# Sukikui/PTI-LDM-VAE

Measured on AMD Instinct MI355X. Metric: vae_train_images_per_sec_256x256, higher is better.
Workload: dtype fp16 forward operands + activations / bf16 backward operands + gradients, fp32 accumulate; 1 GPU; config/vae_dente_no_adv.json 256x256x1 batch 32/GPU: fwd + L1 + 1e-3*KL + bwd + all-reduce + Adam (perceptual term omitted: --perceptual times it; adversarial branch inactive before epoch 6, --adv times it); global_batch=32, parallelism=dp1

## Files before the change

### pti_ldm_vae_amd/csrc/wgrad_mfma.hip

```cpp
#include "pti_common.h"

namespace {

constexpr int TH = 8, TW = 16;
constexpr int PTI_WGRAD_SLAB_V4 = 1 << 30;
#ifndef PTI_WGRAD_BATCH_MAX
#define PTI_WGRAD_BATCH_MAX 16
#endif

struct WgArgs {
  const bf16* x;
  const bf16* dy;
  const stat_t* in_stats;
  const float* gamma;
  const float* beta;
  float* slab;
  int N, H, W, Cin, Ho, Wo, Cout;
  int mode, prologue, groups;
  float eps, inv_cnt;
  int tiles_x, tiles_y, ntiles, S;
  int ci_tiles;
  long long slab_stride;
  int x_f16;
  int diag;
};

template <int KS, int S_, int CO_T, int CI_T>
struct WCfg {
  static constexpr int HH = (TH - 1) * S_ + KS, HW = (TW - 1) * S_ + KS;
  static constexpr int NP = HH * HW;
  static constexpr int KK = KS * KS;
  static constexpr int PA = CI_T * 2 + (CI_T == 64 ? 64 : 0);
  static constexpr int PD = CO_T * 2 + (CO_T == 64 ? 64 : 0);
  static constexpr int NCA = CI_T / 8, NCD = CO_T / 8;
  static constexpr int WCO = CO_T / 32, WCI = CI_T / 32, WPX = 4 / (WCO * WCI);
  static constexpr int A_BYTES = NP * PA, D_BYTES = TH * TW * PD;
  static constexpr int HIT = (NP * NCA + 255) / 256, DIT = (TH * TW * NCD + 255) / 256;
  static constexpr int RED_BYTES = (WPX > 1) ? 32 * 32 * 4 * (WPX - 1) * WCO * WCI : 0;
  static constexpr int LDS_BYTES = (A_BYTES + D_BYTES) > RED_BYTES ? (A_BYTES + D_BYTES) : RED_BYTES;
};

template <int KS, int S_, int CO_T, int CI_T, bool PLAIN>
__global__ __launch_bounds__(256, 2) void wgrad_mfma_kernel(WgArgs a) {
  using C = WCfg<KS, S_, CO_T, CI_T>;
  const int prologue = PLAIN ? PTI_PRO_NONE : a.prologue;
  typedef short v4s __attribute__((ext_vector_type(4)));
  __shared__ __attribute__((aligned(16))) unsigned char smem[C::LDS_BYTES];
  unsigned char* lA = smem;
  unsigned char* lD = smem + C::A_BYTES;

  const int tid = threadIdx.x, lane = tid & 63, wave = tid >> 6;
  const int split = blockIdx.y;
  const int cot = blockIdx.x / a.ci_tiles, cit = blockIdx.x % a.ci_tiles;
  const int wco = wave / (C::WCI * C::WPX), wci = (wave / C::WPX) % C::WCI, wpx = wave % C::WPX;

  const int pad_lo = (a.mode == PTI_CONV_S2PAD) ? 0 : (KS - 1) / 2;
  const bool twox = (a.mode == PTI_CONV_UP2);
  const int VH = twox ? 2 * a.H : a.H, VW = twox ? 2 * a.W : a.W;

  const int g = lane >> 4, q = (lane & 15) >> 2, pp = lane & 3;
  const int pk = 8 * (g >> 1) + q;
  const int chl = 16 * (g & 1) + 4 * pp;
  const int dbase = pk * C::PD + (wco * 32 + chl) * 2;
  const int abase = (pk * S_) * C::PA + (wci * 32 + chl) * 2;

  f32x16 acc[C::KK];
#pragma unroll
  for (int t = 0; t < C::KK; ++t)
#pragma unroll
    for (int r = 0; r < 16; ++r) acc[t][r] = 0.f;

  const int alc = tid % C::NCA, alp = tid / C::NCA;
  constexpr int APSTEP = 256 / C::NCA;
  const int dlc = tid % C::NCD, dlp = tid / C::NCD;
  constexpr int DPSTEP = 256 / C::NCD;
  const int cpg = a.Cin / (a.groups > 0 ? a.groups : 1);
  float bsum[8];
#pragma unroll
  for (int j = 0; j < 8; ++j) bsum[j] = 0.f;

  u32x4 araw[C::HIT], draw[C::DIT];
  bool aok[C::HIT];
  int cur_n = -1;
  float sc[8], sh[8];

  auto issue_loads = [&](int tile) {
    int t = tile;
    const int tx_ = t % a.tiles_x; t /= a.tiles_x;
    const int ty_ = t % a.tiles_y;
    const int n = t / a.tiles_y;
    const int oy0 = ty_ * TH, ox0 = tx_ * TW;
    const int vy0 = oy0 * S_ - pad_lo, vx0 = ox0 * S_ - pad_lo;
#pragma unroll
    for (int it = 0; it < C::HIT; ++it) {
      const int p = alp + it * APSTEP;
      const int hy = p / C::HW, hx = p - hy * C::HW;
      const int vy = vy0 + hy, vx = vx0 + hx;
      const bool v = (p < C::NP) && vy >= 0 && vy < VH && vx >= 0 && vx < VW;
      const int iy = twox ? (vy >> 1) : vy, ix = twox ? (vx >> 1) : vx;
      aok[it] = v;
      araw[it] = u32x4{0u, 0u, 0u, 0u};
      if (v) araw[it] = *(const u32x4*)(a.x + ((size_t)(n * a.H + iy) * a.W + ix) * a.Cin + cit * CI_T + alc * 8);
    }
#pragma unroll
    for (int it = 0; it < C::DIT; ++it) {
      const int p = dlp + it * DPSTEP;
      const int ty = p / TW, tx = p % TW;
      const int oy = oy0 + ty, ox = ox0 + tx;
      draw[it] = u32x4{0u, 0u, 0u, 0u};
      if (p < TH * TW && oy < a.Ho && ox < a.Wo)
        draw[it] = *(const u32x4*)(a.dy + ((size_t)(n * a.Ho + oy) * a.Wo + ox) * a.Cout + cot * CO_T + dlc * 8);
    }
    return n;
  };

  auto write_lds = [&](int n) {
    if (prologue != PTI_PRO_NONE && n != cur_n) {
      cur_n = n;
#pragma unroll
      for (int j = 0; j < 8; ++j) {
        const int ch = cit * CI_T + alc * 8 + j;
        const int gg = ch / cpg;
        const float sum = stat_f(a.in_stats, (n * a.groups + gg) * 2), sq = stat_f(a.in_stats, (n * a.groups + gg) * 2 + 1);
        const float mean = sum * a.inv_cnt;
        const float rstd = rsqrtf(fmaxf(sq * a.inv_cnt - mean * mean, 0.f) + a.eps);
        sc[j] = rstd * a.gamma[ch];
        sh[j] = a.beta[ch] - mean * sc[j];
      }
    }
#pragma unroll
    for (int it = 0; it < C::HIT; ++it) {
      const int p = alp + it * APSTEP;
      if (p < C::NP) {
        u32x4 r = araw[it];
        if (prologue != PTI_PRO_NONE && aok[it]) {
          float f[8];
          unpack8f(r, f, a.x_f16);
#pragma unroll
          for (int j = 0; j < 8; ++j) {
            float v = f[j] * sc[j] + sh[j];
            if (prologue == PTI_PRO_GN_SILU) v = silu_f(v);
            f[j] = v;
          }
          r = pack8(f);
        } else if (a.x_f16) {
          float f[8];
          unpack8f(r, f, true);
          r = pack8(f);
        }
        *(u32x4*)(lA + p * C::PA + alc * 16) = r;
      }
    }
#pragma unroll
    for (int it = 0; it < C::DIT; ++it) {
      const int p = dlp + it * DPSTEP;
      if (p < TH * TW) {
        *(u32x4*)(lD + p * C::PD + dlc * 16) = draw[it];
        if (cit == 0) {
          float f[8];
          unpack8(draw[it], f);
#pragma unroll
          for (int j = 0; j < 8; ++j) bsum[j] += f[j];
        }
      }
    }
  };

  int tile = split;
  int n_next = -1;
  if (tile < a.ntiles) n_next = issue_loads(tile);
  for (; tile < a.ntiles; tile += a.S) {
    write_lds(n_next);
    __syncthreads();
    const int nxt = tile + a.S;
    if (nxt < a.ntiles) n_next = issue_loads(nxt);
#pragma unroll
    for (int rr = 0; rr < TH / C::WPX; ++rr) {
      const int row = wpx + rr * C::WPX;
      const unsigned char* dptr = lD + dbase + row * TW * C::PD;
      const v4s d0 = __builtin_amdgcn_ds_read_tr16_b64_v4i16((v4s __attribute__((address_space(3)))*)(dptr));
      const v4s d1 = __builtin_amdgcn_ds_read_tr16_b64_v4i16((v4s __attribute__((address_space(3)))*)(dptr + 4 * C::PD));
      bf16x8 dfrag;
      {
        typedef short v8s __attribute__((ext_vector_type(8)));
        v8s t8 = {d0[0], d0[1], d0[2], d0[3], d1[0], d1[1], d1[2], d1[3]};
        dfrag = __builtin_bit_cast(bf16x8, t8);
      }
#pragma unroll
      for (int kh = 0; kh < KS; ++kh) {
#pragma unroll
        for (int kw = 0; kw < KS; ++kw) {
          const unsigned char* aptr = lA + abase + ((row * S_ + kh) * C::HW + kw) * C::PA;
          const v4s a0 = __builtin_amdgcn_ds_read_tr16_b64_v4i16((v4s __attribute__((address_space(3)))*)(aptr));
          const v4s a1 = __builtin_amdgcn_ds_read_tr16_b64_v4i16((v4s __attribute__((address_space(3)))*)(aptr + 4 * S_ * C::PA));
          typedef short v8s __attribute__((ext_vector_type(8)));
          v8s t8 = {a0[0], a0[1], a0[2], a0[3], a1[0], a1[1], a1[2], a1[3]};
          const bf16x8 afrag = __builtin_bit_cast(bf16x8, t8);
          acc[kh * KS + kw] = __builtin_amdgcn_mfma_f32_32x32x16_bf16(dfrag, afrag, acc[kh * KS + kw], 0, 0, 0);
        }
      }
    }
    __syncthreads();
  }

  float* slab = a.slab + (size_t)split * a.slab_stride;
  const int ci = cit * CI_T + wci * 32 + (lane & 31);
  const int hsel = lane >> 5;
  float* red = reinterpret_cast<float*>(smem);
#pragma unroll
  for (int t = 0; t < C::KK; ++t) {
    if constexpr (C::WPX > 1) {
      if (wpx > 0) {
        float* dst = red + (((wco * C::WCI + wci) * (C::WPX - 1) + (wpx - 1)) * 16) * 64;
#pragma unroll
        for (int r = 0; r < 16; ++r) dst[r * 64 + lane] = acc[t][r];
      }
      __syncthreads();
      if (wpx == 0) {
#pragma unroll
        for (int o = 0; o < C::WPX - 1; ++o) {
          const float* src = red + (((wco * C::WCI + wci) * (C::WPX - 1) + o) * 16) * 64;
#pragma unroll
          for (int r = 0; r < 16; ++r) acc[t][r] += src[r * 64 + lane];
        }
      }
      __syncthreads();
    }
    if (wpx == 0) {
#pragma unroll
      for (int r = 0; r < 16; ++r) {
        const int co = cot * CO_T + wco * 32 + (r & 3) + 8 * (r >> 2) + 4 * hsel;
        slab[((size_t)t * a.Cout + co) * a.Cin + ci] = acc[t][r];
      }
    }
  }
  if (cit == 0) {
    __syncthreads();
#pragma unroll
    for (int j = 0; j < 8; ++j) red[j * 256 + tid] = bsum[j];
    __syncthreads();
    if (tid < CO_T) {
      const int lc = tid / 8, j = tid % 8;
      float s = 0.f;
      for (int k = lc; k < 256; k += C::NCD) s += red[j * 256 + k];
      slab[(size_t)C::KK * a.Cout * a.Cin + cot * CO_T + tid] = s;
    }
  }
}

template <int COB>
struct W3Cfg {
  static constexpr int TH = 8, HH = TH + 2, HW = TW + 2, NP = HH * HW;
  static constexpr int PP = 64;
  static constexpr int A_BYTES = NP * PP, DP_BYTES = TH * TW * PP;
  static constexpr int D_BYTES = COB * DP_BYTES;
  static constexpr int NT = 192;
  static constexpr int DPC = 4 * COB;
  static constexpr int HIT = (NP * 4 + NT - 1) / NT, DIT = (TH * TW * DPC + NT - 1) / NT;
  static constexpr int LDS_BYTES = A_BYTES + D_BYTES;
};

template <int COB, bool PLAIN>
__global__ __launch_bounds__(192) __attribute__((amdgpu_waves_per_eu(COB == 1 ? (PLAIN ? 4 : 3) : 2, COB == 1 ? (PLAIN ? 4 : 3) : 2)))
void wgrad_mfma3_kernel(WgArgs a) {
  using C = W3Cfg<COB>;
  const int prologue = PLAIN ? PTI_PRO_NONE : a.prologue;
  const bool x_f16 = (bool)a.x_f16;
  typedef short v4s __attribute__((ext_vector_type(4)));
  typedef short v8s __attribute__((ext_vector_type(8)));
  __shared__ __attribute__((aligned(16))) unsigned char smem[C::LDS_BYTES];
  unsigned char* lA = smem;
  unsigned char* lD = smem + C::A_BYTES;
  const int tid = threadIdx.x, lane = tid & 63, kw = tid >> 6;
  int split, cc;
  {
    const int id = blockIdx.x, tiles_cc = a.ci_tiles * (a.Cout / (32 * COB));
    if (a.S >= 8) {
      const int k = id >> 3;
      cc = k % tiles_cc;
      split = (k / tiles_cc) * 8 + (id & 7);
    } else {
      cc = id / a.S;
      split = id % a.S;
    }
  }
  const int cot = cc / a.ci_tiles, cit = cc % a.ci_tiles;
  const int co0 = cot * 32 * COB;
  const bool twox = (a.mode == PTI_CONV_UP2);
  const int VH = twox ? 2 * a.H : a.H, VW = twox ? 2 * a.W : a.W;

  const int g = lane >> 4, q = (lane & 15) >> 2, pp = lane & 3;
  const int pk = 8 * (g >> 1) + q, chl = 16 * (g & 1) + 4 * pp;
  const int fbase = pk * C::PP + chl * 2;

  f32x16 acc[COB][3];
#pragma unroll
  for (int h = 0; h < COB; ++h)
#pragma unroll
    for (int t = 0; t < 3; ++t)
#pragma unroll
      for (int r = 0; r < 16; ++r) acc[h][t][r] = 0.f;
  float bsum[8];
#pragma unroll
  for (int j = 0; j < 8; ++j) bsum[j] = 0.f;

  const int lc = tid & 3, lp = tid >> 2;
  const int lcd = tid % C::DPC, lpd = tid / C::DPC;
  constexpr int PSTEP = C::NT / 4, DSTEP = C::NT / C::DPC;
  const int cpg = a.Cin / (a.groups > 0 ? a.groups : 1);
  int cur_n = -1;
  float sc[8], sh[8];
  u32x4 araw[C::HIT], draw[C::DIT];
  unsigned aokm = 0;

  auto issue = [&](int tile) -> int {
    int t = tile;
    const int tx_ = t % a.tiles_x; t /= a.tiles_x;
    const int ty_ = t % a.tiles_y;
    const int n = t / a.tiles_y;
    const int oy0 = ty_ * C::TH, ox0 = tx_ * TW;
#pragma unroll
    for (int it = 0; it < C::HIT; ++it) {
      const int p = lp + it * PSTEP;
      const int hy = p / C::HW, hx = p - hy * C::HW;
      const int vy = oy0 - 1 + hy, vx = ox0 - 1 + hx;
      const bool v = (p < C::NP) && vy >= 0 && vy < VH && vx >= 0 && vx < VW;
      const int iy = twox ? (vy >> 1) : vy, ix = twox ? (vx >> 1) : vx;
      aokm = (aokm & ~(1u << it)) | ((unsigned)v << it);
      araw[it] = u32x4{0u, 0u, 0u, 0u};
      if (v) araw[it] = *(const u32x4*)(a.x + ((size_t)(n * a.H + iy) * a.W + ix) * a.Cin + cit * 32 + lc * 8);
    }
#pragma unroll
    for (int it = 0; it < C::DIT; ++it) {
      const int p = lpd + it * DSTEP;
      const int oy = oy0 + p / TW, ox = ox0 + p % TW;
      draw[it] = u32x4{0u, 0u, 0u, 0u};
      if (p < C::TH * TW && oy < a.Ho && ox < a.Wo)
        draw[it] = *(const u32x4*)(a.dy + ((size_t)(n * a.Ho + oy) * a.Wo + ox) * a.Cout + co0 + lcd * 8);
    }
    return n;
  };
  auto commit = [&](int n) {
    if (prologue != PTI_PRO_NONE && n != cur_n) {
      cur_n = n;
#pragma unroll
      for (int j = 0; j < 8; ++j) {
        const int ch = cit * 32 + lc * 8 + j;
        const int gg = ch / cpg;
        const float sum = stat_f(a.in_stats, (n * a.groups + gg) * 2), sq = stat_f(a.in_stats, (n * a.groups + gg) * 2 + 1);
        const float mean = sum * a.inv_cnt;
        const float rstd = rsqrtf(fmaxf(sq * a.inv_cnt - mean * mean, 0.f) + a.eps);
        sc[j] = rstd * a.gamma[ch];
        sh[j] = a.beta[ch] - mean * sc[j];
      }
    }
#pragma unroll
    for (int it = 0; it < C::HIT; ++it) {
      const int p = lp + it * PSTEP;
      if (p < C::NP) {
        u32x4 r = araw[it];
        if (prologue != PTI_PRO_NONE && ((aokm >> it) & 1u)) {
          float f[8];
          unpack8f(r, f, x_f16);
#pragma unroll
          for (int j = 0; j < 8; ++j) {
            float v = f[j] * sc[j] + sh[j];
            if (prologue == PTI_PRO_GN_SILU) v = silu_f(v);
            f[j] = v;
          }
          r = pack8(f);
        } else if (x_f16) {
          float f[8];
          unpack8f(r, f, true);
          r = pack8(f);
        }
        *(u32x4*)(lA + p * C::PP + lc * 16) = r;
      }
    }
#pragma unroll
    for (int it = 0; it < C::DIT; ++it) {
      const int p = lpd + it * DSTEP;
      if (p < C::TH * TW) {
        *(u32x4*)(lD + (lcd >> 2) * C::DP_BYTES + p * C::PP + (lcd & 3) * 16) = draw[it];
        if (cit == 0) {
          float f[8];
          unpack8(draw[it], f);
#pragma unroll
          for (int j = 0; j < 8; ++j) bsum[j] += f[j];
        }
      }
    }
  };

  int tile = split, n_next = -1;
  if (tile < a.ntiles) n_next = issue(tile);
  for (; tile < a.ntiles; tile += a.S) {
    commit(n_next);
    __syncthreads();
    const int nxt = tile + a.S;
    if (nxt < a.ntiles) n_next = issue(nxt);
// ... 771 lines not shown
#pragma unroll
    for (int r = 0; r < 4; ++r) dfr[r] = dnx[r];
    ps = ns;
  }
  wait_vmcnt<0>();

  const int ci = lane & 31, hsel = lane >> 5;
  if (do_bias) bsum += __shfl_xor(bsum, 32, 64);
  if constexpr (C::NRG == 2) {
    __syncthreads();
    float* red = reinterpret_cast<float*>(smem) + (cb + C::NCB * ch) * 5120;
    float* bred = reinterpret_cast<float*>(smem) + C::NCB * C::NCH * 5120;
#pragma unroll
    for (int round = 0; round < 2; ++round) {
      if (round) __syncthreads();
      if (rg == 1) {
#pragma unroll
        for (int t = 0; t < 9; ++t)
          if ((t < 5) == (round == 0))
#pragma unroll
            for (int q4 = 0; q4 < 4; ++q4)
              *(f32x4*)(red + (t - 5 * round) * 1024 + ci * 32 + (((2 * q4 + hsel) ^ (ci & 7)) << 2)) =
                  f32x4{acc[t / 3][t % 3][4 * q4], acc[t / 3][t % 3][4 * q4 + 1], acc[t / 3][t % 3][4 * q4 + 2], acc[t / 3][t % 3][4 * q4 + 3]};
        if (round == 0 && do_bias && lane < 32) bred[cb * 32 + lane] = bsum;
      }
      __syncthreads();
      if (rg == 0) {
#pragma unroll
        for (int t = 0; t < 9; ++t)
          if ((t < 5) == (round == 0))
#pragma unroll
            for (int q4 = 0; q4 < 4; ++q4) {
              const f32x4 v = *(const f32x4*)(red + (t - 5 * round) * 1024 + ci * 32 + (((2 * q4 + hsel) ^ (ci & 7)) << 2));
#pragma unroll
              for (int j = 0; j < 4; ++j) acc[t / 3][t % 3][4 * q4 + j] += v[j];
            }
        if (round == 0 && do_bias && lane < 32) bsum += bred[cb * 32 + lane];
      }
    }
    if (rg == 1) return;
  }
  const int cc32 = (C::NCB * cotb + cb) * (a.Cin / 32) + C::NCH * citb + ch;
  float* blk = a.slab + (size_t)split * a.slab_stride + (size_t)cc32 * 9216;
#pragma unroll
  for (int kh = 0; kh < 3; ++kh)
#pragma unroll
    for (int kw = 0; kw < 3; ++kw)
#pragma unroll
      for (int q4 = 0; q4 < 4; ++q4)
        *(f32x4*)(blk + (kh * 3 + kw) * 1024 + ci * 32 + (((2 * q4 + hsel) ^ (ci & 7)) << 2)) =
            f32x4{acc[kh][kw][4 * q4], acc[kh][kw][4 * q4 + 1], acc[kh][kw][4 * q4 + 2], acc[kh][kw][4 * q4 + 3]};
  if (do_bias && lane < 32) a.slab[(size_t)split * a.slab_stride + (size_t)9 * a.Cout * a.Cin + co0 + cb * 32 + lane] = bsum;
}

__global__ __launch_bounds__(256) void wgrad_reduce4_kernel(W4Batch b) {
  __shared__ f32x4 red[16][16];
  int jb = 0;
  while (jb + 1 < b.njobs && (int)blockIdx.x >= b.first_rblk[jb + 1]) ++jb;
  const W4Job& a = b.job[jb];
  const float* __restrict__ slab = a.slab;
  float* __restrict__ dw = b.dw[jb];
  float* __restrict__ dbias = b.dbias[jb];
  const int S = a.S, Cout = a.Cout, Cin = a.Cin, accumulate = b.accumulate[jb];
  const long long stride = a.slab_stride;
  const long long total = (long long)9 * Cout * Cin;
  const int col = threadIdx.x & 15, sg = threadIdx.x >> 4;
  const long long e = ((long long)(blockIdx.x - b.first_rblk[jb]) * 16 + col) * 4;
  f32x4 s0 = {0.f, 0.f, 0.f, 0.f}, s1 = s0;
  if (e < total + Cout) {
    int k = sg;
    for (; k + 16 < S; k += 32) {
      s0 += *(const f32x4*)(slab + (size_t)k * stride + e);
      s1 += *(const f32x4*)(slab + (size_t)(k + 16) * stride + e);
    }
    if (k < S) s0 += *(const f32x4*)(slab + (size_t)k * stride + e);
  }
  red[sg][col] = s0 + s1;
  __syncthreads();
  if (sg == 0 && e < total + Cout) {
    f32x4 sum = red[0][col];
#pragma unroll
    for (int g = 1; g < 16; ++g) sum += red[g][col];
    if (e < total) {
      const int cc = (int)(e / 9216), i = (int)(e % 9216);
      const int ci_tiles = Cin / 32;
      const int co0 = (cc / ci_tiles) * 32, ci0 = (cc % ci_tiles) * 32;
      const int tap = i >> 10, ci = (i >> 5) & 31, cog = ((i >> 2) & 7) ^ (ci & 7);
#pragma unroll
      for (int j = 0; j < 4; ++j) {
        const size_t o = ((size_t)(co0 + cog * 4 + j) * Cin + ci0 + ci) * 9 + tap;
        dw[o] = accumulate ? dw[o] + sum[j] : sum[j];
      }
    } else if (dbias) {
      const int co = (int)(e - total);
#pragma unroll
      for (int j = 0; j < 4; ++j) dbias[co + j] = accumulate ? dbias[co + j] + sum[j] : sum[j];
    }
  }
}

__global__ __launch_bounds__(256) void wgrad_reduce_kernel(const float* __restrict__ slab, long long stride, int S,
                                                           float* __restrict__ dw, float* __restrict__ dbias, int Cout,
                                                           int Cin, int KK, int accumulate) {
  __shared__ f32x4 red[16][16];
  const long long total = (long long)KK * Cout * Cin;
  const int col = threadIdx.x & 15, sg = threadIdx.x >> 4;
  const long long e = ((long long)blockIdx.x * 16 + col) * 4;
  f32x4 s0 = {0.f, 0.f, 0.f, 0.f}, s1 = s0;
  if (e < total + Cout) {
    int k = sg;
    for (; k + 16 < S; k += 32) {
      s0 += *(const f32x4*)(slab + (size_t)k * stride + e);
      s1 += *(const f32x4*)(slab + (size_t)(k + 16) * stride + e);
    }
    if (k < S) s0 += *(const f32x4*)(slab + (size_t)k * stride + e);
  }
  red[sg][col] = s0 + s1;
  __syncthreads();
  if (sg == 0 && e < total + Cout) {
    f32x4 sum = red[0][col];
#pragma unroll
    for (int g = 1; g < 16; ++g) sum += red[g][col];
    if (e < total) {
      const int ci = e % Cin;
      const int co = (e / Cin) % Cout;
      const int t = e / ((long long)Cin * Cout);
#pragma unroll
      for (int j = 0; j < 4; ++j) {
        const size_t o = ((size_t)co * Cin + ci + j) * KK + t;
        dw[o] = accumulate ? dw[o] + sum[j] : sum[j];
      }
    } else if (dbias) {
      const int co = (int)(e - total);
#pragma unroll
      for (int j = 0; j < 4; ++j) dbias[co + j] = accumulate ? dbias[co + j] + sum[j] : sum[j];
    }
  }
}

template <int KS, int S_, int CO_T, int CI_T>
void launch_w(const WgArgs& a, int grid_y, hipStream_t st) {
  if (a.prologue == PTI_PRO_NONE)
    PTI_LAUNCH((wgrad_mfma_kernel<KS, S_, CO_T, CI_T, true>), dim3(grid_y, a.S), dim3(256), 0, st, a);
  else
    PTI_LAUNCH((wgrad_mfma_kernel<KS, S_, CO_T, CI_T, false>), dim3(grid_y, a.S), dim3(256), 0, st, a);
}
template <int KS, int S_>
void launch_wt(const WgArgs& a, int co_t, int ci_t, int grid_y, hipStream_t st) {
  if (co_t == 64 && ci_t == 64) launch_w<KS, S_, 64, 64>(a, grid_y, st);
  else if (co_t == 64) launch_w<KS, S_, 64, 32>(a, grid_y, st);
  else if (ci_t == 64) launch_w<KS, S_, 32, 64>(a, grid_y, st);
  else launch_w<KS, S_, 32, 32>(a, grid_y, st);
}

}

static int w6_mode(int n, int h, int w, int cin, int cout) {
  const char* e = getenv("PTI_WGRAD_V6");
  const int v = e ? atoi(e) : 3;
  if (v >= 1 && cout % 128 == 0 && cin % 64 == 0) return 2;
  if (v >= 2 && cout % 64 == 0 && cin % 64 == 0 && (v == 2 || (long long)h * w <= 128 * 128)) return 3;
  return 0;
}
static void w4_fill_job(W4Job& a, const void* x, const void* dy, int n, int h, int w, int cin, int cout, int mode) {
  a.x = (const bf16*)x; a.dy = (const bf16*)dy; a.slab = nullptr;
  a.N = n; a.H = h; a.W = w; a.Cin = cin; a.Cout = cout;
  a.tiles_x = cdiv(w, TW); a.tiles_y = cdiv(h, mode == 2 ? W6A::TH_ : TH); a.ntiles = n * a.tiles_x * a.tiles_y;
  a.slab_stride = (long long)9 * cout * cin + cout;
  a.S = 1;
  a.cob2 = mode;
}
static bool w4_eligible(int n, int h, int w, int cin, int cout) {
  return n > 0 && h > 0 && w > 0 && cin > 0 && cout > 0 && cin % 32 == 0 && cout % 32 == 0 &&
         (long long)n * h * w * cin * 2 < (1ll << 31) && (long long)n * h * w * cout * 2 < (1ll << 31);
}
static int w4_mode(int cout) {
  static const int cob2_env = getenv("PTI_WGRAD_V4_COB2") ? atoi(getenv("PTI_WGRAD_V4_COB2")) : 1;
  return (cob2_env && cout % 64 == 0) ? 1 : 0;
}
extern "C" int pti_conv_wgrad_batched_mode(int n, int h, int w, int cin, int cout) {
  if (!w4_eligible(n, h, w, cin, cout)) return PTI_EUNSUPPORTED;
  const int v4 = w4_mode(cout), v6 = w6_mode(n, h, w, cin, cout);
  return v6 ? v6 : v4;
}
static int wgrad_diag_env() {
  const char* v = getenv("PTI_WGRAD_V4_DIAG");
  const char* ok = getenv("PTI_ALLOW_WRONG_RESULTS");
  if (!v || atoi(v) == 0) return 0;
  if (!ok || atoi(ok) != 1) {
    fprintf(stderr, "[pti] PTI_WGRAD_V4_DIAG ignored: it needs PTI_ALLOW_WRONG_RESULTS=1 (results are garbage)\n");
    return 0;
  }
  fprintf(stderr, "[pti] WRONG-RESULT DIAGNOSTIC ACTIVE: PTI_WGRAD_V4_DIAG=%s\n", v);
  return atoi(v);
}
static long long w4_plan(W4Batch& b, float* workspace, long long workspace_floats) {
  static const int wgs_env = getenv("PTI_WGRAD_V4_WGS") ? atoi(getenv("PTI_WGRAD_V4_WGS")) : 2048;
  static const int diag_env = wgrad_diag_env();
  b.diag = diag_env;
  auto tiles32 = [](const W4Job& a) {
    return a.cob2 == 2 ? (a.Cin / 64) * (a.Cout / 128) : a.cob2 == 3 ? (a.Cin / 64) * (a.Cout / 64)
                                                                     : (a.Cin / 32) * (a.Cout / (a.cob2 ? 64 : 32));
  };
  const bool m6 = b.njobs > 0 && b.job[0].cob2 >= 2;
  const char* w6e = getenv("PTI_WGRAD_V6_WGS");
  const int wgs6 = w6e && atoi(w6e) > 0 ? atoi(w6e) : 512;
  double work = 0;
  for (int j = 0; j < b.njobs; ++j) work += (double)tiles32(b.job[j]) * (b.job[j].cob2 == 1 ? 2 : 1) * b.job[j].ntiles;
  double per_wg = work / wgs_env > 2.0 ? work / wgs_env : 2.0;
  if (m6) per_wg = work / wgs6 > 4.0 ? work / wgs6 : 4.0;
  for (int attempt = 0;; ++attempt) {
    long long used = 0;
    int rb = 0, groups = 0;
    bool fits = true;
    for (int j = 0; j < b.njobs; ++j) {
      W4Job& a = b.job[j];
      int S = (int)((double)a.ntiles * (a.cob2 == 1 ? 2 : 1) / per_wg + 0.5);
      if (S > a.ntiles / (a.cob2 ? 1 : 2)) S = a.ntiles / (a.cob2 ? 1 : 2);
      if (S > 255) S = 255;
      if (S < 1) S = 1;
      if (used + (long long)S * a.slab_stride > workspace_floats) fits = false;
      a.S = S;
      a.slab = workspace + used;
      used += (long long)S * a.slab_stride;
      groups += S;
      b.first_rblk[j] = rb;
      rb += (int)((a.slab_stride / 4 + 15) / 16);
    }
    b.first_rblk[b.njobs] = rb;
    if (fits && groups <= 8 * W4_MAXGRP) {
      int len[8] = {0, 0, 0, 0, 0, 0, 0, 0};
      for (int x = 0; x < 8; ++x) { b.ngrp[x] = 0; b.grp_start[x][0] = 0; }
      int order[PTI_WGRAD_BATCH_MAX];
      for (int j = 0; j < b.njobs; ++j) order[j] = j;
      for (int i = 0; i < b.njobs; ++i)
        for (int j = i + 1; j < b.njobs; ++j)
          if (tiles32(b.job[order[j]]) > tiles32(b.job[order[i]])) { const int t = order[i]; order[i] = order[j]; order[j] = t; }
      bool ok = true;
      for (int i = 0; i < b.njobs && ok; ++i) {
        const int j = order[i];
        for (int sp = 0; sp < b.job[j].S; ++sp) {
          int best = 0;
          for (int x = 1; x < 8; ++x)
            if (len[x] < len[best]) best = x;
          if (b.ngrp[best] >= W4_MAXGRP || len[best] + tiles32(b.job[j]) > 65535) { ok = false; break; }
          b.grp[best][b.ngrp[best]] = (unsigned short)((unsigned)j | ((unsigned)sp << 4));
          len[best] += tiles32(b.job[j]);
          b.grp_start[best][++b.ngrp[best]] = (unsigned short)len[best];
        }
      }
      if (ok) {
        int mx = 0;
        for (int x = 0; x < 8; ++x) mx = len[x] > mx ? len[x] : mx;
        b.nwg = 8 * mx;
        return used;
      }
    }
    if (attempt > 40) return -1;
    per_wg *= 1.25;
  }
}

extern "C" int64_t pti_conv_wgrad_workspace_bytes(int cout, int cin, int ksize, int splits) {
  return (int64_t)splits * ((int64_t)ksize * ksize * cout * cin + cout) * 4;
}

static int wgrad_check(const void* x, const void* dy, const int64_t* in_stats, const float* gamma, const float* beta,
                       const void* workspace, const pti_conv_desc* d) {
  if (!x || !dy || !workspace || !d) PTI_FAIL(PTI_EINVAL, "conv_wgrad_mfma: null pointer");
  if (d->cin % 32 || d->cout % 32) PTI_FAIL(PTI_EUNSUPPORTED, "conv_wgrad_mfma: cin=%d cout=%d", d->cin, d->cout);
  if (d->ksize != 1 && d->ksize != 3) PTI_FAIL(PTI_EUNSUPPORTED, "conv_wgrad_mfma: ksize");
  if (d->mode == PTI_CONV_ZINS || (d->ksize == 1 && d->mode != PTI_CONV_S1)) PTI_FAIL(PTI_EUNSUPPORTED, "conv_wgrad_mfma: mode %d", d->mode);
  if (d->prologue != PTI_PRO_NONE && (!in_stats || !gamma || !beta || d->groups <= 0 || d->cin % d->groups))
    PTI_FAIL(PTI_EINVAL, "conv_wgrad_mfma: prologue args");
  return PTI_OK;
}

extern "C" int pti_conv_wgrad_mfma_partials(const void* x, const void* dy, const int64_t* in_stats, const float* gamma,
                                            const float* beta, void* workspace, int64_t workspace_bytes,
                                            const pti_conv_desc* d, int* splits_out, pti_stream_t s) {
  if (!splits_out) PTI_FAIL(PTI_EINVAL, "conv_wgrad_mfma_partials: null splits_out");
  if (int rc = wgrad_check(x, dy, in_stats, gamma, beta, workspace, d)) return rc;
  WgArgs a;
  a.x = (const bf16*)x; a.dy = (const bf16*)dy; a.in_stats = (const stat_t*)in_stats; a.gamma = gamma; a.beta = beta;
  a.slab = (float*)workspace;
  a.N = d->n; a.H = d->h; a.W = d->w; a.Cin = d->cin; a.Ho = d->ho; a.Wo = d->wo; a.Cout = d->cout;
  a.mode = d->mode; a.prologue = d->prologue; a.groups = d->groups; a.eps = d->eps; a.x_f16 = d->in_f16;
  static const int diag_env = wgrad_diag_env();
  a.diag = diag_env;
  a.inv_cnt = d->prologue != PTI_PRO_NONE ? 1.0f / ((float)(d->cin / d->groups) * (float)d->h * (float)d->w) : 0.f;
  a.tiles_x = cdiv(d->wo, TW); a.tiles_y = cdiv(d->ho, TH); a.ntiles = d->n * a.tiles_x * a.tiles_y;
  int co_t = d->cout % 64 == 0 ? 64 : 32, ci_t = d->cin % 64 == 0 ? 64 : 32;
  if ((long long)a.ntiles * (d->cout / co_t) * (d->cin / ci_t) < 16 * 512) co_t = ci_t = 32;
  const bool v3 = d->ksize == 3 && d->mode != PTI_CONV_S2PAD;
  static const int cob_env = getenv("PTI_WGRAD_COB") ? atoi(getenv("PTI_WGRAD_COB")) : 0;
  const bool cob_ok = d->cout % 64 == 0 && d->mode == PTI_CONV_S1;
  const int cob = (cob_ok && cob_env != 1 && (cob_env == 2 || d->prologue != PTI_PRO_NONE)) ? 2 : 1;
  if (v3) { ci_t = 32; co_t = 32 * cob; }
  a.ci_tiles = d->cin / ci_t;
  const int tiles_cc = (d->cout / co_t) * a.ci_tiles;
  const int kk = d->ksize * d->ksize;
  a.slab_stride = (long long)kk * d->cout * d->cin + d->cout;
  const long long smax = workspace_bytes / (a.slab_stride * 4);
  const bool plain = d->prologue == PTI_PRO_NONE && cob == 1;
  static const int v1_wgs = getenv("PTI_WGRAD_V1_WGS") ? atoi(getenv("PTI_WGRAD_V1_WGS")) : 512;
  int S = (v3 ? (cob == 2 ? 512 : (plain ? (tiles_cc == 1 ? 1024 : 1280) : 768)) : v1_wgs) / tiles_cc;
  if (S > a.ntiles / 4) S = a.ntiles / 4;
  const int scap = v3 ? (plain ? 1024 : 512) : 256;
  if (S > scap) S = scap;
  if (S < 1) S = 1;
  if (S > smax) S = (int)smax;
  if (S < 1) PTI_FAIL(PTI_EINVAL, "conv_wgrad_mfma: workspace too small (%lld bytes per split needed)", a.slab_stride * 4);
  static const int v4_env = getenv("PTI_WGRAD_V4") ? atoi(getenv("PTI_WGRAD_V4")) : 1;
  const bool v4 = v3 && v4_env && d->prologue == PTI_PRO_NONE && !d->in_f16 && d->mode == PTI_CONV_S1 &&
                  w4_eligible(d->n, d->h, d->w, d->cin, d->cout);
  if (v4) {
    W4Batch b;
    b.njobs = 1;
    w4_fill_job(b.job[0], x, dy, d->n, d->h, d->w, d->cin, d->cout, pti_conv_wgrad_batched_mode(d->n, d->h, d->w, d->cin, d->cout));
    b.dw[0] = b.dbias[0] = nullptr;
    b.accumulate[0] = 0;
    if (w4_plan(b, (float*)workspace, workspace_bytes / 4) < 0)
      PTI_FAIL(PTI_EINVAL, "conv_wgrad_mfma: workspace too small (%lld bytes per split needed)", a.slab_stride * 4);
    const char* v5e = getenv("PTI_WGRAD_V5");
    const bool v5 = v5e && atoi(v5e) != 0 && !b.diag;
    if (b.job[0].cob2 == 2) PTI_LAUNCH(wgrad_mfma6_kernel<W6A>, dim3(b.nwg), dim3(512), 0, (hipStream_t)s, b);
    else if (b.job[0].cob2 == 3) PTI_LAUNCH(wgrad_mfma6_kernel<W6B>, dim3(b.nwg), dim3(512), 0, (hipStream_t)s, b);
    else if (b.job[0].cob2 && v5) PTI_LAUNCH(wgrad_mfma5_kernel, dim3(b.nwg), dim3(256), 0, (hipStream_t)s, b);
    else if (b.job[0].cob2) PTI_LAUNCH(wgrad_mfma4_kernel<true>, dim3(b.nwg), dim3(512), 0, (hipStream_t)s, b);
    else PTI_LAUNCH(wgrad_mfma4_kernel<false>, dim3(b.nwg), dim3(512), 0, (hipStream_t)s, b);
    PTI_CHECK_LAUNCH("conv_wgrad_mfma");
    *splits_out = b.job[0].S | PTI_WGRAD_SLAB_V4;
    return PTI_OK;
  }
  if (v3 && S >= 8) S &= ~7;
  a.S = S;
  hipStream_t st = (hipStream_t)s;
  if (v3 && cob == 2) PTI_LAUNCH((wgrad_mfma3_kernel<2, false>), dim3(tiles_cc * S), dim3(192), 0, st, a);
  else if (v3 && plain) PTI_LAUNCH((wgrad_mfma3_kernel<1, true>), dim3(tiles_cc * S), dim3(192), 0, st, a);
  else if (v3) PTI_LAUNCH((wgrad_mfma3_kernel<1, false>), dim3(tiles_cc * S), dim3(192), 0, st, a);
  else if (d->ksize == 1) launch_wt<1, 1>(a, co_t, ci_t, tiles_cc, st);
  else launch_wt<3, 2>(a, co_t, ci_t, tiles_cc, st);
  PTI_CHECK_LAUNCH("conv_wgrad_mfma");
  *splits_out = S;
  return PTI_OK;
}

extern "C" int pti_conv_wgrad_reduce(const void* workspace, int splits, float* dw, float* dbias, int accumulate,
                                     const pti_conv_desc* d, pti_stream_t s) {
  if (!workspace || !dw || !d || splits < 1) PTI_FAIL(PTI_EINVAL, "conv_wgrad_reduce: bad arguments");
  const int kk = d->ksize * d->ksize;
  const long long total = (long long)kk * d->cout * d->cin + d->cout;
  if (splits & PTI_WGRAD_SLAB_V4) {
    if (kk != 9 || !w4_eligible(d->n, d->h, d->w, d->cin, d->cout)) PTI_FAIL(PTI_EINVAL, "conv_wgrad_reduce: block-ordered slabs are 3x3 only");
    W4Batch b;
    b.njobs = 1;
    w4_fill_job(b.job[0], nullptr, nullptr, d->n, d->h, d->w, d->cin, d->cout, w4_mode(d->cout));
    b.job[0].S = splits & ~PTI_WGRAD_SLAB_V4;
    b.job[0].slab = (float*)workspace;
    b.dw[0] = dw; b.dbias[0] = dbias; b.accumulate[0] = accumulate;
    b.diag = 0; b.nwg = 0;
    for (int x = 0; x < 8; ++x) b.ngrp[x] = 0;
    b.first_rblk[0] = 0;
    b.first_rblk[1] = (int)((total / 4 + 15) / 16);
    PTI_LAUNCH(wgrad_reduce4_kernel, dim3(b.first_rblk[1]), dim3(256), 0, (hipStream_t)s, b);
    PTI_CHECK_LAUNCH("conv_wgrad_reduce");
    return PTI_OK;
  }
  PTI_LAUNCH(wgrad_reduce_kernel, dim3((unsigned)((total / 4 + 15) / 16)), dim3(256), 0, (hipStream_t)s,
                     (const float*)workspace, total, splits, dw, dbias, d->cout, d->cin, kk, accumulate);
  PTI_CHECK_LAUNCH("conv_wgrad_reduce");
  return PTI_OK;
}

extern "C" int pti_conv_wgrad_mfma(const void* x, const void* dy, const int64_t* in_stats, const float* gamma,
                                   const float* beta, float* dw, float* dbias, void* workspace,
                                   int64_t workspace_bytes, int accumulate, const pti_conv_desc* d, pti_stream_t s) {
  if (!dw) PTI_FAIL(PTI_EINVAL, "conv_wgrad_mfma: null pointer");
  int splits = 0;
  if (int rc = pti_conv_wgrad_mfma_partials(x, dy, in_stats, gamma, beta, workspace, workspace_bytes, d, &splits, s)) return rc;
  return pti_conv_wgrad_reduce(workspace, splits, dw, dbias, accumulate, d, s);
}

extern "C" int pti_conv_wgrad_mfma_batched(const pti_wgrad_job* jobs, int njobs, void* workspace, int64_t workspace_bytes,
                                           pti_stream_t s) {
  if (!jobs || !workspace || njobs < 1 || njobs > PTI_WGRAD_BATCH_MAX)
    PTI_FAIL(PTI_EINVAL, "conv_wgrad_mfma_batched: 1..%d jobs", PTI_WGRAD_BATCH_MAX);
  W4Batch bm[4];
  bm[0].njobs = bm[1].njobs = bm[2].njobs = bm[3].njobs = 0;
  for (int j = 0; j < njobs; ++j) {
    const pti_wgrad_job& q = jobs[j];
    if (!q.x || !q.dy || !q.dw) PTI_FAIL(PTI_EINVAL, "conv_wgrad_mfma_batched: job %d has a null pointer", j);
    const int mode = pti_conv_wgrad_batched_mode(q.n, q.h, q.w, q.cin, q.cout);
    if (mode < 0)
      PTI_FAIL(PTI_EUNSUPPORTED, "conv_wgrad_mfma_batched: job %d: n=%d h=%d w=%d cin=%d cout=%d (channels must be multiples of 32, tensors < 2 GiB)",
               j, q.n, q.h, q.w, q.cin, q.cout);
    W4Job jb;
    w4_fill_job(jb, q.x, q.dy, q.n, q.h, q.w, q.cin, q.cout, mode);
    W4Batch& b = bm[mode];
    const int k = b.njobs++;
    b.job[k] = jb;
    b.dw[k] = q.dw; b.dbias[k] = q.dbias; b.accumulate[k] = q.accumulate;
  }
  float* ws = (float*)workspace;
  long long ws_floats = workspace_bytes / 4;
  const char* v5e = getenv("PTI_WGRAD_V5");
  const int v5_env = v5e ? atoi(v5e) : 0;
  const void* main_kernel = nullptr;
  long long need[4] = {0, 0, 0, 0}, need_all = 0;
  for (int m = 0; m < 4; ++m) {
    for (int j = 0; j < bm[m].njobs; ++j) need[m] += bm[m].job[j].slab_stride;
    need_all += need[m];
  }
  if (need_all > ws_floats) PTI_FAIL(PTI_EINVAL, "conv_wgrad_mfma_batched: workspace too small (%lld bytes needed for one split per job)", need_all * 4);
  const long long ws_total = ws_floats;
  for (int m = 3; m >= 0; --m) {
    W4Batch& b = bm[m];
    if (b.njobs == 0) continue;
    long long later = 0;
    for (int m2 = m - 1; m2 >= 0; --m2) later += need[m2];
    long long avail = (long long)((double)ws_total * ((double)need[m] / (double)need_all));
    if (avail < need[m]) avail = need[m];
    if (later == 0 || avail > ws_floats - later) avail = ws_floats - later;
    const long long used = w4_plan(b, ws, avail);
    if (used < 0) PTI_FAIL(PTI_EINVAL, "conv_wgrad_mfma_batched: workspace too small");
    ws += used;
    ws_floats -= used;
    const void* kfn;
    if (m == 3) { PTI_LAUNCH(wgrad_mfma6_kernel<W6B>, dim3(b.nwg), dim3(512), 0, (hipStream_t)s, b); kfn = reinterpret_cast<const void*>(wgrad_mfma6_kernel<W6B>); }
    else if (m == 2) { PTI_LAUNCH(wgrad_mfma6_kernel<W6A>, dim3(b.nwg), dim3(512), 0, (hipStream_t)s, b); kfn = reinterpret_cast<const void*>(wgrad_mfma6_kernel<W6A>); }
    else if (m == 1 && v5_env && !b.diag) { PTI_LAUNCH(wgrad_mfma5_kernel, dim3(b.nwg), dim3(256), 0, (hipStream_t)s, b); kfn = reinterpret_cast<const void*>(wgrad_mfma5_kernel); }
    else if (m == 1) { PTI_LAUNCH(wgrad_mfma4_kernel<true>, dim3(b.nwg), dim3(512), 0, (hipStream_t)s, b); kfn = reinterpret_cast<const void*>(wgrad_mfma4_kernel<true>); }
    else { PTI_LAUNCH(wgrad_mfma4_kernel<false>, dim3(b.nwg), dim3(512), 0, (hipStream_t)s, b); kfn = reinterpret_cast<const void*>(wgrad_mfma4_kernel<false>); }
    PTI_CHECK_LAUNCH("conv_wgrad_mfma_batched");
    if (!main_kernel) main_kernel = kfn;
    PTI_LAUNCH(wgrad_reduce4_kernel, dim3(b.first_rblk[b.njobs]), dim3(256), 0, (hipStream_t)s, b);
    PTI_CHECK_LAUNCH("conv_wgrad_mfma_batched reduce");
  }
  pti_last_kernel = main_kernel;
  return PTI_OK;
}
```

Baseline: 2739 images/s.

## Add dedicated 1x1 weight-gradient kernel with pixel-linear tiles and larger channel tiles

```diff
diff --git a/pti_ldm_vae_amd/csrc/wgrad_mfma.hip b/pti_ldm_vae_amd/csrc/wgrad_mfma.hip
--- a/pti_ldm_vae_amd/csrc/wgrad_mfma.hip
+++ b/pti_ldm_vae_amd/csrc/wgrad_mfma.hip
@@ -1,3 +1,5 @@
+#include <algorithm>
+
 #include "pti_common.h"
 
 namespace {
@@ -41,7 +43,7 @@
 };
 
 template <int KS, int S_, int CO_T, int CI_T, bool PLAIN>
-__global__ __launch_bounds__(256, 2) void wgrad_mfma_kernel(WgArgs a) {
+__device__ __forceinline__ void wgrad_v1_body(const WgArgs& a) {
   using C = WCfg<KS, S_, CO_T, CI_T>;
   const int prologue = PLAIN ? PTI_PRO_NONE : a.prologue;
   typedef short v4s __attribute__((ext_vector_type(4)));
@@ -246,6 +248,229 @@
       slab[(size_t)C::KK * a.Cout * a.Cin + cot * CO_T + tid] = s;
     }
   }
+}
+
+constexpr int w1_tile_pixels(int co_t, int ci_t) { return co_t + ci_t <= 128 ? 128 : (co_t + ci_t <= 320 ? 64 : 32); }
+
+template <int CO_T, int CI_T>
+struct W1Cfg {
+  static constexpr int NBCO = CO_T / 32, NBCI = CI_T / 32;
+  static constexpr int WCO = (NBCO >= 4 && NBCI == 1) ? 4 : (NBCO >= 2 ? 2 : 1);
+  static constexpr int WCI = (NBCI >= 4 && NBCO == 1) ? 4 : (NBCI >= 2 ? 2 : 1);
+  static constexpr int WPX = 4 / (WCO * WCI);
+  static constexpr int BCO = NBCO / WCO, BCI = NBCI / WCI;
+  static constexpr int P = w1_tile_pixels(CO_T, CI_T);
+  static constexpr int NCA = CI_T / 8, NCD = CO_T / 8;
+  static constexpr int AIT = P * NCA / 256, DIT = P * NCD / 256;
+  static constexpr int skew(int nb) { return nb >= 4 ? 64 : (nb == 2 ? 128 : 0); }
+  static constexpr int SUBX = P * 64 + skew(NBCI), SUBD = P * 64 + skew(NBCO);
+  static constexpr int X_BYTES = NBCI * SUBX, D_BYTES = NBCO * SUBD;
+  static constexpr int RED_BYTES = (WPX > 1) ? 32 * 32 * 4 * (WPX - 1) * WCO * WCI : 0;
+  static constexpr int BIAS_BYTES = 8 * 256 * 4;
+  static constexpr int TILE_BYTES = X_BYTES + D_BYTES;
+  static constexpr int LDS_BYTES = TILE_BYTES > (RED_BYTES > BIAS_BYTES ? RED_BYTES : BIAS_BYTES)
+                                       ? TILE_BYTES : (RED_BYTES > BIAS_BYTES ? RED_BYTES : BIAS_BYTES);
+  static_assert(WCO * WCI * WPX == 4 && BCO * WCO == NBCO && BCI * WCI == NBCI, "wave layout");
+  static_assert(WPX == 1 || (BCO == 1 && BCI == 1), "waves split pixels only when each holds one block");
+  static_assert(P % (16 * WPX) == 0 && (P * NCA) % 256 == 0 && (P * NCD) % 256 == 0 && 256 % NCA == 0 && 256 % NCD == 0,
+                "loader geometry");
+};
+
+template <int CO_T, int CI_T, bool PLAIN>
+__device__ __forceinline__ void wgrad_1x1_body(const WgArgs& a) {
+  using C = W1Cfg<CO_T, CI_T>;
+  const int prologue = PLAIN ? PTI_PRO_NONE : a.prologue;
+  typedef short v4s __attribute__((ext_vector_type(4)));
+  typedef short v8s __attribute__((ext_vector_type(8)));
+  __shared__ __attribute__((aligned(16))) unsigned char smem[C::LDS_BYTES];
+  unsigned char* lX = smem;
+  unsigned char* lD = smem + C::X_BYTES;
+
+  const int tid = threadIdx.x, lane = tid & 63, wave = tid >> 6;
+  const int split = blockIdx.y;
+  const int cot = blockIdx.x / a.ci_tiles, cit = blockIdx.x % a.ci_tiles;
+  const int wco = wave / (C::WCI * C::WPX), wci = (wave / C::WPX) % C::WCI, wpx = wave % C::WPX;
+  const int HW = a.H * a.W;
+  const int tps = a.tiles_x;
+  const int t0 = (int)((long long)split * a.ntiles / a.S), t1 = (int)((long long)(split + 1) * a.ntiles / a.S);
+
+  const int g = lane >> 4, q = (lane & 15) >> 2, pp = lane & 3;
+  const int fbase = (8 * (g >> 1) + q) * 64 + (16 * (g & 1) + 4 * pp) * 2;
+
+  f32x16 acc[C::BCO * C::BCI];
+#pragma unroll
+  for (int b = 0; b < C::BCO * C::BCI; ++b)
+#pragma unroll
+    for (int r = 0; r < 16; ++r) acc[b][r] = 0.f;
+
+  constexpr int APSTEP = 256 / C::NCA, DPSTEP = 256 / C::NCD;
+  const int alc = tid % C::NCA, alp = tid / C::NCA;
+  const int dlc = tid % C::NCD, dlp = tid / C::NCD;
+  const bf16* xg = a.x + cit * CI_T + alc * 8;
+  const bf16* dg = a.dy + cot * CO_T + dlc * 8;
+  unsigned char* xl = lX + (alc >> 2) * C::SUBX + (alc & 3) * 16 + alp * 64;
+  unsigned char* dl = lD + (dlc >> 2) * C::SUBD + (dlc & 3) * 16 + dlp * 64;
+  const int cpg = a.Cin / (a.groups > 0 ? a.groups : 1);
+  float bsum[8];
+#pragma unroll
+  for (int j = 0; j < 8; ++j) bsum[j] = 0.f;
+
+  u32x4 araw[C::AIT], draw[C::DIT];
+  int cur_n = -1, n_next = -1, valid_next = 0;
+  float sc[8], sh[8];
+
+  auto issue_loads = [&](int tile) {
+    const int n = tile / tps, p0 = (tile - n * tps) * C::P;
+    const int valid = min(C::P, HW - p0);
+    const size_t pix0 = (size_t)n * HW + p0;
+#pragma unroll
+    for (int it = 0; it < C::AIT; ++it) {
+      const int p = alp + it * APSTEP;
+      araw[it] = u32x4{0u, 0u, 0u, 0u};
+      if (p < valid) araw[it] = *(const u32x4*)(xg + (pix0 + p) * a.Cin);
+    }
+#pragma unroll
+    for (int it = 0; it < C::DIT; ++it) {
+      const int p = dlp + it * DPSTEP;
+      draw[it] = u32x4{0u, 0u, 0u, 0u};
+      if (p < valid) draw[it] = *(const u32x4*)(dg + (pix0 + p) * a.Cout);
+    }
+    n_next = n;
+    valid_next = valid;
+  };
+
+  auto write_lds = [&]() {
+    if (prologue != PTI_PRO_NONE && n_next != cur_n) {
+      cur_n = n_next;
+#pragma unroll
+      for (int j = 0; j < 8; ++j) {
+        const int ch = cit * CI_T + alc * 8 + j;
+        const int gg = ch / cpg;
+        const float sum = stat_f(a.in_stats, (cur_n * a.groups + gg) * 2), sq = stat_f(a.in_stats, (cur_n * a.groups + gg) * 2 + 1);
+        const float mean = sum * a.inv_cnt;
+        const float rstd = rsqrtf(fmaxf(sq * a.inv_cnt - mean * mean, 0.f) + a.eps);
+        sc[j] = rstd * a.gamma[ch];
+        sh[j] = a.beta[ch] - mean * sc[j];
+      }
+    }
+#pragma unroll
+    for (int it = 0; it < C::AIT; ++it) {
+      u32x4 r = araw[it];
+      if (prologue != PTI_PRO_NONE) {
+        if (alp + it * APSTEP < valid_next) {
+          float f[8];
+          unpack8f(r, f, a.x_f16);
+#pragma unroll
+          for (int j = 0; j < 8; ++j) {
+            float v = f[j] * sc[j] + sh[j];
+            if (prologue == PTI_PRO_GN_SILU) v = silu_f(v);
+            f[j] = v;
+          }
+          r = pack8(f);
+        }
+      } else if (a.x_f16) {
+        float f[8];
+        unpack8f(r, f, true);
+        r = pack8(f);
+      }
+      *(u32x4*)(xl + it * APSTEP * 64) = r;
+    }
+#pragma unroll
+    for (int it = 0; it < C::DIT; ++it) {
+      *(u32x4*)(dl + it * DPSTEP * 64) = draw[it];
+      if (cit == 0) {
+        float f[8];
+        unpack8(draw[it], f);
+#pragma unroll
+        for (int j = 0; j < 8; ++j) bsum[j] += f[j];
+      }
+    }
+  };
+
+  if (t0 < t1) issue_loads(t0);
+  for (int tile = t0; tile < t1; ++tile) {
+    write_lds();
+    __syncthreads();
+    if (tile + 1 < t1) issue_loads(tile + 1);
+#pragma unroll
+    for (int ks = 0; ks < C::P / 16 / C::WPX; ++ks) {
+      const int poff = (ks * C::WPX + wpx) * 16 * 64 + fbase;
+      bf16x8 dfrag[C::BCO], xfrag[C::BCI];
+#pragma unroll
+      for (int i = 0; i < C::BCO; ++i) {
+        const unsigned char* ptr = lD + (wco * C::BCO + i) * C::SUBD + poff;
+        const v4s d0 = __builtin_amdgcn_ds_read_tr16_b64_v4i16((v4s __attribute__((address_space(3)))*)(ptr));
+        const v4s d1 = __builtin_amdgcn_ds_read_tr16_b64_v4i16((v4s __attribute__((address_space(3)))*)(ptr + 4 * 64));
+        const v8s t8 = {d0[0], d0[1], d0[2], d0[3], d1[0], d1[1], d1[2], d1[3]};
+        dfrag[i] = __builtin_bit_cast(bf16x8, t8);
+      }
+#pragma unroll
+      for (int j = 0; j < C::BCI; ++j) {
+        const unsigned char* ptr = lX + (wci * C::BCI + j) * C::SUBX + poff;
+        const v4s x0 = __builtin_amdgcn_ds_read_tr16_b64_v4i16((v4s __attribute__((address_space(3)))*)(ptr));
+        const v4s x1 = __builtin_amdgcn_ds_read_tr16_b64_v4i16((v4s __attribute__((address_space(3)))*)(ptr + 4 * 64));
+        const v8s t8 = {x0[0], x0[1], x0[2], x0[3], x1[0], x1[1], x1[2], x1[3]};
+        xfrag[j] = __builtin_bit_cast(bf16x8, t8);
+      }
+#pragma unroll
+      for (int i = 0; i < C::BCO; ++i)
+#pragma unroll
+        for (int j = 0; j < C::BCI; ++j)
+          acc[i * C::BCI + j] = __builtin_amdgcn_mfma_f32_32x32x16_bf16(dfrag[i], xfrag[j], acc[i * C::BCI + j], 0, 0, 0);
+    }
+    __syncthreads();
+  }
+
+  float* slab = a.slab + (size_t)split * a.slab_stride;
+  const int hsel = lane >> 5;
+  float* red = reinterpret_cast<float*>(smem);
+  if constexpr (C::WPX > 1) {
+    if (wpx > 0) {
+      float* dst = red + (((wco * C::WCI + wci) * (C::WPX - 1) + (wpx - 1)) * 16) * 64;
+#pragma unroll
+      for (int r = 0; r < 16; ++r) dst[r * 64 + lane] = acc[0][r];
+    }
+    __syncthreads();
+    if (wpx == 0) {
+#pragma unroll
+      for (int o = 0; o < C::WPX - 1; ++o) {
+        const float* src = red + (((wco * C::WCI + wci) * (C::WPX - 1) + o) * 16) * 64;
+#pragma unroll
+        for (int r = 0; r < 16; ++r) acc[0][r] += src[r * 64 + lane];
+      }
+    }
+  }
+  if (wpx == 0) {
+#pragma unroll
+    for (int i = 0; i < C::BCO; ++i)
+#pragma unroll
+      for (int j = 0; j < C::BCI; ++j) {
+        const int ci = cit * CI_T + (wci * C::BCI + j) * 32 + (lane & 31);
+#pragma unroll
+        for (int r = 0; r < 16; ++r) {
+          const int co = cot * CO_T + (wco * C::BCO + i) * 32 + (r & 3) + 8 * (r >> 2) + 4 * hsel;
+          slab[(size_t)co * a.Cin + ci] = acc[i * C::BCI + j][r];
+        }
+      }
+  }
+  if (cit == 0) {
+    __syncthreads();
+#pragma unroll
+    for (int j = 0; j < 8; ++j) red[j * 256 + tid] = bsum[j];
+    __syncthreads();
+    if (tid < CO_T) {
+      const int lc = tid / 8, j = tid % 8;
+      float s = 0.f;
+      for (int k = lc; k < 256; k += C::NCD) s += red[j * 256 + k];
+      slab[(size_t)a.Cout * a.Cin + cot * CO_T + tid] = s;
+    }
+  }
+}
+
+template <int KS, int S_, int CO_T, int CI_T, bool PLAIN>
+__global__ __launch_bounds__(256, 2) void wgrad_mfma_kernel(WgArgs a) {
+  if constexpr (KS == 1 && S_ == 1) wgrad_1x1_body<CO_T, CI_T, PLAIN>(a);
+  else wgrad_v1_body<KS, S_, CO_T, CI_T, PLAIN>(a);
 }
 
 template <int COB>
@@ -1323,6 +1548,12 @@
   else if (ci_t == 64) launch_w<KS, S_, 32, 64>(a, grid_y, st);
   else launch_w<KS, S_, 32, 32>(a, grid_y, st);
 }
+template <int CI_T>
+void launch_w1(const WgArgs& a, int co_t, int grid_y, hipStream_t st) {
+  if (co_t == 128) launch_w<1, 1, 128, CI_T>(a, grid_y, st);
+  else if (co_t == 64) launch_w<1, 1, 64, CI_T>(a, grid_y, st);
+  else launch_w<1, 1, 32, CI_T>(a, grid_y, st);
+}
 
 }
 
@@ -1447,6 +1678,40 @@
   return PTI_OK;
 }
 
+static int v1_wgs_env() {
+  static const int v = getenv("PTI_WGRAD_V1_WGS") ? atoi(getenv("PTI_WGRAD_V1_WGS")) : 512;
+  return v;
+}
+
+static int wgrad_1x1_launch(WgArgs& a, const pti_conv_desc* d, int64_t workspace_bytes, int* splits_out, pti_stream_t s) {
+  const int ci_t = d->cin % 256 == 0 ? 256 : d->cin % 128 == 0 ? 128 : d->cin % 64 == 0 ? 64 : 32;
+  const int co_t = d->cout % 128 == 0 ? 128 : d->cout % 64 == 0 ? 64 : 32;
+  const int P = w1_tile_pixels(co_t, ci_t);
+  const long long hw = (long long)d->h * d->w;
+  a.tiles_x = (int)((hw + P - 1) / P); a.tiles_y = 1; a.ntiles = d->n * a.tiles_x;
+  a.ci_tiles = d->cin / ci_t;
+  const int groups = (d->cout / co_t) * a.ci_tiles;
+  a.slab_stride = (long long)d->cout * d->cin + d->cout;
+  const long long slab_bytes = a.slab_stride * 4;
+  const long long operand_bytes = 2 * d->n * hw * (d->cin + d->cout);
+  long long S = v1_wgs_env() / groups;
+  S = std::min(S, (long long)d->n * cdiv(d->h, 4) * cdiv(d->w, 16));
+  S = std::min(S, (long long)a.ntiles);
+  S = std::min(S, operand_bytes / (2 * slab_bytes));
+  S = std::max(S, 1ll);
+  S = std::min(S, (long long)(workspace_bytes / slab_bytes));
+  if (S < 1) PTI_FAIL(PTI_EINVAL, "conv_wgrad_mfma: workspace too small (%lld bytes per split needed)", slab_bytes);
+  a.S = (int)S;
+  hipStream_t st = (hipStream_t)s;
+  if (ci_t == 256) launch_w1<256>(a, co_t, groups, st);
+  else if (ci_t == 128) launch_w1<128>(a, co_t, groups, st);
+  else if (ci_t == 64) launch_w1<64>(a, co_t, groups, st);
+  else launch_w1<32>(a, co_t, groups, st);
+  PTI_CHECK_LAUNCH("conv_wgrad_mfma");
+  *splits_out = a.S;
+  return PTI_OK;
+}
+
 extern "C" int pti_conv_wgrad_mfma_partials(const void* x, const void* dy, const int64_t* in_stats, const float* gamma,
                                             const float* beta, void* workspace, int64_t workspace_bytes,
                                             const pti_conv_desc* d, int* splits_out, pti_stream_t s) {
@@ -1460,6 +1725,7 @@
   static const int diag_env = wgrad_diag_env();
   a.diag = diag_env;
   a.inv_cnt = d->prologue != PTI_PRO_NONE ? 1.0f / ((float)(d->cin / d->groups) * (float)d->h * (float)d->w) : 0.f;
+  if (d->ksize == 1) return wgrad_1x1_launch(a, d, workspace_bytes, splits_out, s);
   a.tiles_x = cdiv(d->wo, TW); a.tiles_y = cdiv(d->ho, TH); a.ntiles = d->n * a.tiles_x * a.tiles_y;
   int co_t = d->cout % 64 == 0 ? 64 : 32, ci_t = d->cin % 64 == 0 ? 64 : 32;
   if ((long long)a.ntiles * (d->cout / co_t) * (d->cin / ci_t) < 16 * 512) co_t = ci_t = 32;
@@ -1474,7 +1740,7 @@
   a.slab_stride = (long long)kk * d->cout * d->cin + d->cout;
   const long long smax = workspace_bytes / (a.slab_stride * 4);
   const bool plain = d->prologue == PTI_PRO_NONE && cob == 1;
-  static const int v1_wgs = getenv("PTI_WGRAD_V1_WGS") ? atoi(getenv("PTI_WGRAD_V1_WGS")) : 512;
+  const int v1_wgs = v1_wgs_env();
   int S = (v3 ? (cob == 2 ? 512 : (plain ? (tiles_cc == 1 ? 1024 : 1280) : 768)) : v1_wgs) / tiles_cc;
   if (S > a.ntiles / 4) S = a.ntiles / 4;
   const int scap = v3 ? (plain ? 1024 : 512) : 256;
@@ -1510,7 +1776,6 @@
   if (v3 && cob == 2) PTI_LAUNCH((wgrad_mfma3_kernel<2, false>), dim3(tiles_cc * S), dim3(192), 0, st, a);
   else if (v3 && plain) PTI_LAUNCH((wgrad_mfma3_kernel<1, true>), dim3(tiles_cc * S), dim3(192), 0, st, a);
   else if (v3) PTI_LAUNCH((wgrad_mfma3_kernel<1, false>), dim3(tiles_cc * S), dim3(192), 0, st, a);
-  else if (d->ksize == 1) launch_wt<1, 1>(a, co_t, ci_t, tiles_cc, st);
   else launch_wt<3, 2>(a, co_t, ci_t, tiles_cc, st);
   PTI_CHECK_LAUNCH("conv_wgrad_mfma");
   *splits_out = S;
```

Result: no change. 2758 images/s (median of 6 runs) (+0.7%).
